# Alisah-Ozcan/HEonGPU

Measured on AMD Instinct MI355X. Metric: homomorphic mults/sec (CKKS N=2^16, L=16) + NTT GB/s vs HBM roofline, higher is better.
Workload: dtype u64

## Files before the change

heongpu_amd/csrc/ntt.hip:

```cpp
#include "ntt.hpp"
#define HEGPU_FP_TU ntt
#include "fpmod.cuh"

namespace hegpu {

#define NTT_THREADS 256

#ifdef NTT_ABLATION_HEADER
#include NTT_ABLATION_HEADER
#else
__device__ __forceinline__ u64 gld(const u64* p) { return *p; }
__device__ __forceinline__ void gst(u64* p, u64 v) { *p = v; }
#define NTT_ABLATE_BFLY(x, y, w)
#define NTT_ABLATE_FPBFLY(x, y, w)
#define NTT_ABLATE_TW(load, root0, s) (load)
#define NTT_FP_TW(t, i, c) ((t)[i])
#endif

__device__ __forceinline__ u64 csub(u64 x, u64 m) { return (x >= m) ? x - m : x; }

typedef unsigned long long u64x2_t __attribute__((ext_vector_type(2)));
struct ConstTw {
    const u64x2_t __attribute__((address_space(4)))* p;
    __device__ __forceinline__ ulonglong2 operator[](u32 i) const
// ... 883 lines not shown
            x[2 * k + 1] = v.y;
        }
        ct_radix16_tb<LAZY>(x, tb, qc);
        if (LAZY) {
#pragma unroll
            for (int k = 0; k < 16; k++) r[k] = reduce64(x[k], md);
        } else {
#pragma unroll
            for (int k = 0; k < 16; k++) r[k] = csub(csub(csub(x[k], qc.q4), 2 * qc.q), qc.q);
        }
    }
    wave_lds_fence();
#pragma unroll
    for (int k = 0; k < 8; k++)
        *reinterpret_cast<ulonglong2*>(&lds[row_phys(row * 256 + 16 * i0 + 2 * k)]) = make_ulonglong2(r[2 * k], r[2 * k + 1]);
    wave_lds_fence();
    row_store_all(a, ps, md, a.out + ps.out_off, (u64) g * 4096 + row * 256 + i0, lds, row, i0);
}

template <int S1, bool DECOMP = false>
__global__ __launch_bounds__(16 << S1, 4) void ntt_fwd_single(NttArgs a)
{
    extern __shared__ __attribute__((aligned(16))) u64 limb[];
    const PolySel ps = select_poly(a, blockIdx.x);
    if (DECOMP && a.skip_identity && ps.mod == ps.digit) return;
    const Mod md = a.mods[ps.mod];
    if (md.fp) fwd_single_body<S1, true, false, DECOMP>(a, ps, md, limb);
    else if (fwd_stages_lazy(md, a.lazy_q_max)) fwd_single_body<S1, false, true, DECOMP>(a, ps, md, limb);
    else fwd_single_body<S1, false, false, DECOMP>(a, ps, md, limb);
}

static_assert(ks_unreduced_exit(16, 60) == 16 && ks_unreduced_exit(17, 60) == 12 && ks_unreduced_exit(21, 60) == 12, "");
static_assert(ks_unreduced_exit(22, 60) == 8 && ks_unreduced_exit(32, 60) == 8 && ks_unreduced_exit(33, 60) == 0, "");
static_assert(ks_unreduced_exit(4, 61) == 16 && ks_unreduced_exit(8, 61) == 8 && ks_unreduced_exit(9, 61) == 0, "");

template <bool LAZY, int ROOM = 8, int EXIT = 0>
__device__ __forceinline__ void ks_row_digit(u64 (&x)[16], const u64* __restrict__ p, u64* lds,
                                             const ulonglong2* twa, const ulonglong2* __restrict__ tb,
                                             const QC& qc, const Mod& md, int row, int i0)
{
    static_assert(EXIT == 0 || (!LAZY && (EXIT == 8 || ((EXIT == 12 || EXIT == 16) && ROOM == 16))), "exit bound");
    constexpr CsSched CS = cs_sched(8, ROOM, EXIT ? EXIT : 8);
#pragma unroll
    for (int k = 0; k < 16; k++) x[k] = gld(&p[row * 256 + i0 + 16 * k]);
#pragma unroll
    for (int s = 0; s < 4; s++) {
        const int half = 8 >> s;
        const int cs = LAZY ? 0 : (int) (((CS.c8 >> s) & 1u) * 2u + ((CS.c4 >> s) & 1u));
#pragma unroll
        for (int b = 0; b < (1 << s); b++) {
            const ulonglong2 w = twa[((1 << s) - 1 + b) * 16 + row];
#pragma unroll
            for (int j = 0; j < half; j++) ct_bfly_cs(x[b * 2 * half + j], x[b * 2 * half + j + half], w, qc, cs);
        }
    }
#pragma unroll
    for (int k = 0; k < 16; k++) lds[row_phys(row * 256 + i0 + 16 * k)] = x[k];
    wave_lds_fence();
#pragma unroll
    for (int k = 0; k < 8; k++) {
        ulonglong2 v = *reinterpret_cast<const ulonglong2*>(&lds[row_phys(row * 256 + 16 * i0 + 2 * k)]);
        x[2 * k] = v.x;
        x[2 * k + 1] = v.y;
    }
    ct_radix16_tb<LAZY, (CS.c8 >> 4), (CS.c4 >> 4)>(x, tb, qc);
    if (!LAZY && EXIT == 0) {
#pragma unroll
        for (int k = 0; k < 16; k++) x[k] = csub(csub(csub(x[k], qc.q4), 2 * qc.q), qc.q);
    }
    wave_lds_fence();
#pragma unroll
    for (int k = 0; k < 8; k++)
        *reinterpret_cast<ulonglong2*>(&lds[row_phys(row * 256 + 16 * i0 + 2 * k)]) =
            make_ulonglong2(x[2 * k], x[2 * k + 1]);
    wave_lds_fence();
#pragma unroll
    for (int k = 0; k < 16; k++) x[k] = lds[row_phys(row * 256 + i0 + 16 * k)];
    wave_lds_fence();
}

struct KsIdx { int item, tile, slot; bool valid; int d0, d1; };
__host__ __device__ __forceinline__ unsigned ks_slots(const KsMacArgs& a, int kind)
{
    const int all = a.slot_count ? a.slot_count : a.rc;
    if (a.int_slot_count <= 0 || kind == 0) return (unsigned) all;
    return kind == 1 ? (unsigned) a.int_slot_count : (unsigned) (all - a.int_slot_count);
}
template <bool SPLIT, int KIND = 0>
__device__ __forceinline__ KsIdx ks_index(const KsMacArgs& a)
{
    const unsigned b = blockIdx.x, xcd = b & 7u, j = b >> 3;
    const unsigned splits = SPLIT ? (unsigned) a.splits : 1u;
    const unsigned units = (unsigned) a.items * splits;
    const unsigned tiles = 1u << (a.n_power - 12);
    const unsigned total = ks_slots(a, KIND) * tiles * units, chunk = (total + 7u) >> 3;
    const unsigned lin = xcd * chunk + j;
    const unsigned g = lin / units, unit = lin - g * units;
    const unsigned item = SPLIT ? unit / splits : unit, sp = SPLIT ? unit - item * splits : 0u;
    const unsigned nslots = ks_slots(a, KIND), gt = g / nslots;
    KsIdx r;
    r.valid = lin < total;
    r.item = (int) item;
    r.tile = (int) gt;
    int si = (int) (g - gt * nslots);
    if (KIND == 1 && a.int_slot_count > 0) {
        si = a.int_slots[r.valid ? si : 0];
    } else {
        si += a.slot_first;
        if (KIND == 2 && a.int_slot_count > 0) {
#pragma unroll
            for (int q = 0; q < 8; q++)
                if (q < a.int_slot_count && a.int_slots[q] <= si) si++;
        }
    }
    r.slot = si;
    r.d0 = SPLIT ? (int) (sp * (unsigned) a.digits / splits) : 0;
    r.d1 = SPLIT ? (int) ((sp + 1) * (unsigned) a.digits / splits) : a.digits;
    return r;
}

__device__ __forceinline__ void ks_tail_scatter(const KsMacArgs& a, int item, int slot, int p, u64 e0, const u64 (&r)[16])
{
    const KsMacArgs::Tail& e = a.tail;
    u64* out = e.out + e.out_item_stride * item + ((u64) (p * e.limbs + slot) << a.n_power);
    if (e.galois_inv) {
#pragma unroll
        for (int k = 0; k < 16; k++) {
            const u32 el = (u32) e0 + 16 * k;
            const u32 ex = ((2u * (__brev(el) >> (32 - a.n_power)) + 1u) * e.galois_inv) & ((2u << a.n_power) - 1u);
            out[__brev((ex - 1u) >> 1) >> (32 - a.n_power)] = r[k];
        }
    } else {
#pragma unroll
        for (int k = 0; k < 16; k++) out[e0 + 16 * k] = r[k];
    }
}
__device__ __forceinline__ void ks_tail_store(const KsMacArgs& a, int item, int slot, int p, u64 e0, const Mod& md, u64 inv,
                                              const u64 (&acc)[16], const u64 (&tv)[16], bool with_ct, const u64 (&cv)[16])
{
    u64 r[16];
#pragma unroll
    for (int k = 0; k < 16; k++) r[k] = mul_barrett(sub_mod(acc[k], tv[k], md.q), inv, md);
    if (with_ct) {
#pragma unroll
        for (int k = 0; k < 16; k++) r[k] = add_mod(cv[k], r[k], md.q);
    }
    ks_tail_scatter(a, item, slot, p, e0, r);
}
__device__ __forceinline__ void ks_tail_store_fp(const KsMacArgs& a, int item, int slot, int p, u64 e0, const FC& fc, double inv,
                                                 const double (&acc)[16], const double (&tv)[16], bool with_ct,
                                                 const u64 (&cv)[16])
{
    double m[16];
#pragma unroll
    for (int k = 0; k < 16; k++) {
        FP_STAGE(fc, FP_STAGE_OUT);
        const double d = fp_reduce(acc[k], fc) - tv[k];
        FP_STAGE(fc, FP_STAGE_TAIL);
        FP_AUDIT_VAL(fc, FPM_SUM, d);
        m[k] = fp_mul_nc(d, inv, fc);
    }
    FP_STAGE(fc, FP_STAGE_OUT);
    if (with_ct) {
#pragma unroll
        for (int k = 0; k < 16; k++) m[k] += fp_from_u64(cv[k]);
    }
    u64 r[16];
#pragma unroll
    for (int k = 0; k < 16; k++) r[k] = fp_to_u64(fp_canon(m[k], fc));
    ks_tail_scatter(a, item, slot, p, e0, r);
}
__device__ __forceinline__ const u64* ks_tail_T(const KsMacArgs& a, int item, int slot, int tile, int p)
{
    return a.tail.T + a.tail.T_item_stride * item + ((u64) (p * a.rc + slot) << a.n_power) + (u64) tile * 4096;
}
__device__ __forceinline__ bool ks_tail_ct(const KsMacArgs& a, int item, int slot, int p, u64 e0, u64 (&cv)[16])
{
    const KsMacArgs::Tail& e = a.tail;
    if (!e.ct || (e.ct_parts && p >= e.ct_parts)) return false;
    const u64* c = e.ct + e.ct_item_stride * item + ((u64) (p * e.limbs + slot) << a.n_power) + e0;
#pragma unroll
    for (int k = 0; k < 16; k++) cv[k] = c[16 * k];
    return true;
}

#define KS_TW_LDS_BYTES ((15 * 256 + 15 * 16) * 8)
template <bool SPLIT, bool MD = false>
__device__ __forceinline__ void ks_row_mac_int_body(const KsMacArgs& a, const KsIdx& ki, const Mod& md, int midx,
                                                    u64* lds, void* twbuf)
{
    const int t = threadIdx.x;
    const int item = ki.item, tile = ki.tile, slot = ki.slot;
    const QC qc = make_qc(md.q);
    const int s1 = a.n_power - 8;
    const ulonglong2* __restrict__ tw = a.tw + ((u64) midx << a.n_power);
    const int row = t >> 4, i0 = t & 15;
    const u32 crow = tile * 16 + row;
    const ulonglong2* __restrict__ tb = a.twB + ((u64) midx * (15u << (a.n_power - 4))) + ((u64) crow * 15 * 16 + i0);
    const u64 n = (u64) 1 << a.n_power;
    const u64* __restrict__ pin = a.in + a.in_item_stride * item + ((u64) slot << a.n_power) + (u64) tile * 4096;
    const u64* __restrict__ pk = a.key + ((u64) midx << a.n_power) + (u64) tile * 4096 + row * 256 + i0;
    const u64 dig_off = (u64) a.rc << a.n_power;
    const u64 key_off1 = (u64) a.key_limbs << a.n_power, key_off2 = (u64) a.key_limbs << (a.n_power + 1);
    const bool lazy = row_stages_lazy(md, a.lazy_q_max) && md.q <= ~0ull / (u64) a.digits;
    const bool room16 = stages_room16(md);
    const int ex = a.unreduced_exit;
    ulonglong2* twa = reinterpret_cast<ulonglong2*>(twbuf);
    if (i0 < 15) {
        const int s = (i0 >= 7) ? 3 : (i0 >= 3) ? 2 : (i0 >= 1) ? 1 : 0;
        twa[i0 * 16 + row] = tw[((((u32) 1 << s1) + crow) << s) + (i0 - ((1 << s) - 1))];
    }
    wave_lds_fence();

    const int item_s = MD ? __builtin_amdgcn_readfirstlane(item) : 0, slot_s = MD ? __builtin_amdgcn_readfirstlane(slot) : 0;
    const int tile_s = MD ? __builtin_amdgcn_readfirstlane(tile) : 0, midx_s = MD ? __builtin_amdgcn_readfirstlane(midx) : 0;
    u64 h0[16], l0[16], h1[16], l1[16];
#pragma unroll
    for (int k = 0; k < 16; k++) h0[k] = l0[k] = h1[k] = l1[k] = 0;
    for (int i = ki.d0; i < ki.d1; i++) {
        u64 x[16];
        const u64* p = pin + dig_off * i;
        if (a.skip_identity && i == midx) {
            const u64* pi = a.ident + a.ident_item_stride * item + ((u64) i << a.n_power) + (u64) tile * 4096;
#pragma unroll
            for (int k = 0; k < 16; k++) x[k] = gld(&pi[row * 256 + i0 + 16 * k]);
        } else if (lazy) {
            ks_row_digit<true>(x, p, lds, twa, tb, qc, md, row, i0);
        } else if (room16) {
            if (ex == 16) ks_row_digit<false, 16, 16>(x, p, lds, twa, tb, qc, md, row, i0);
            else if (ex == 12) ks_row_digit<false, 16, 12>(x, p, lds, twa, tb, qc, md, row, i0);
            else if (ex == 8) ks_row_digit<false, 16, 8>(x, p, lds, twa, tb, qc, md, row, i0);
            else ks_row_digit<false, 16>(x, p, lds, twa, tb, qc, md, row, i0);
        } else {
            if (ex) ks_row_digit<false, 8, 8>(x, p, lds, twa, tb, qc, md, row, i0);
            else ks_row_digit<false>(x, p, lds, twa, tb, qc, md, row, i0);
        }
        const u64* k0 = pk + key_off2 * i;
        const u64* k1 = k0 + key_off1;
#pragma unroll
        for (int k = 0; k < 16; k++) {
            acc128(h0[k], l0[k], x[k], k0[16 * k]);
            acc128(h1[k], l1[k], x[k], k1[16 * k]);
        }
    }
    if constexpr (MD) {
        u64 acc0[16], acc1[16];
#pragma unroll
        for (int k = 0; k < 16; k++) {
            acc0[k] = reduce128(h0[k], l0[k], md);
            acc1[k] = reduce128(h1[k], l1[k], md);
        }
        int tt = threadIdx.x;
        asm volatile("" : "+v"(tt));
        const int trow = tt >> 4, ti0 = tt & 15;
        const u64 e0 = (u64) tile_s * 4096 + trow * 256 + ti0;
        const u64 inv = a.tail.inv[midx_s];
        const bool lazy_t = row_stages_lazy(md, a.lazy_q_max);
        const ulonglong2* __restrict__ ttb = a.twB + ((u64) midx_s * (15u << (a.n_power - 4))) + ((u64) (tile_s * 16 + trow) * 15 * 16 + ti0);
        auto part = [&](int p, const u64 (&acc)[16]) {
            u64 cv[16], x[16];
            const bool with_ct = ks_tail_ct(a, item_s, slot_s, p, e0, cv);
            const u64* pT = ks_tail_T(a, item_s, slot_s, tile_s, p);
            if (lazy_t) {
                ks_row_digit<true>(x, pT, lds, twa, ttb, qc, md, trow, ti0);
#pragma unroll
                for (int k = 0; k < 16; k++) x[k] = reduce64(x[k], md);
            } else if (room16) {
                ks_row_digit<false, 16>(x, pT, lds, twa, ttb, qc, md, trow, ti0);
            } else {
                ks_row_digit<false>(x, pT, lds, twa, ttb, qc, md, trow, ti0);
            }
            ks_tail_store(a, item_s, slot_s, p, e0, md, inv, acc, x, with_ct, cv);
        };
        __builtin_amdgcn_sched_barrier(0);
        part(0, acc0);
        __builtin_amdgcn_sched_barrier(0);
        part(1, acc1);
        return;
    }
    u64* po = (SPLIT ? const_cast<u64*>(pin) + dig_off * ki.d0 - (u64) tile * 4096
                     : a.out + a.out_item_stride * item + ((u64) slot << a.n_power)) +
              (u64) tile * 4096 + row * 256 + i0;
#pragma unroll
    for (int k = 0; k < 16; k++) {
        po[16 * k] = reduce128(h0[k], l0[k], md);
        po[dig_off + 16 * k] = reduce128(h1[k], l1[k], md);
    }
    (void) n;
}

template <bool SPLIT>
__global__ __launch_bounds__(NTT_THREADS, SPLIT ? 2 : 1) void ks_row_mac(KsMacArgs a)
{
    __shared__ __attribute__((aligned(16))) u64 lds[ROW_LDS_ELEMS];
    __shared__ ulonglong2 twa[15 * 16];
    const KsIdx ki = ks_index<SPLIT, SPLIT ? 0 : 1>(a);
    if (!ki.valid) return;
    const int midx = a.mod_order ? a.mod_order[ki.slot] : ki.slot;
    const Mod md = a.mods[midx];
    if (md.fp) return;
    ks_row_mac_int_body<SPLIT>(a, ki, md, midx, lds, twa);
}

template <bool SPLIT>
__device__ __forceinline__ void ks_fp_row(double (&x)[16], const u64 (&xr)[16], const double* twl, u64* lds, const FC& fc,
                                          int s1, int row, int i0, int t)
{
    if constexpr (SPLIT) {
#pragma unroll
        for (int k = 0; k < 16; k++) x[k] = as_f64(xr[k]);
#pragma unroll
        for (int s = 0; s < 4; s++) {
            const int half = 8 >> s;
            FP_STAGE(fc, s1 + s);
#pragma unroll
            for (int b = 0; b < (1 << s); b++) {
                const double w = twl[15 * 256 + ((1 << s) - 1 + b) * 16 + row];
#pragma unroll
                for (int j = 0; j < half; j++) fp_ct_bfly(x[b * 2 * half + j], x[b * 2 * half + j + half], w, fc);
            }
        }
        FP_STAGE(fc, s1 + 4);
#pragma unroll
        for (int k = 0; k < 16; k++) x[k] = fp_reduce(x[k], fc);
#pragma unroll
        for (int k = 0; k < 16; k++) lds[row_phys(row * 256 + i0 + 16 * k)] = as_bits(x[k]);
        wave_lds_fence();
#pragma unroll
        for (int k = 0; k < 8; k++) {
            ulonglong2 v = *reinterpret_cast<const ulonglong2*>(&lds[row_phys(row * 256 + 16 * i0 + 2 * k)]);
            x[2 * k] = as_f64(v.x);
            x[2 * k + 1] = as_f64(v.y);
        }
#pragma unroll
        for (int s = 0; s < 4; s++) {
            const int half = 8 >> s;
            FP_STAGE(fc, s1 + 4 + s);
#pragma unroll
            for (int b = 0; b < (1 << s); b++) {
                const double w = twl[((1 << s) - 1 + b) * 256 + t];
#pragma unroll
                for (int j = 0; j < half; j++) fp_ct_bfly(x[b * 2 * half + j], x[b * 2 * half + j + half], w, fc);
            }
        }
    } else {
        int row_o = row, t_o = t;
        asm volatile("" : "+v"(row_o), "+v"(t_o));
        const double* twa = twl + 15 * 256 + row_o;
        const double* twb = twl + t_o;
        double wn[8], wc[8];
        wc[0] = twa[0];
        wn[0] = twa[16];
        wn[1] = twa[32];
        __builtin_amdgcn_sched_barrier(0);
#pragma unroll
        for (int k = 0; k < 16; k++) x[k] = as_f64(xr[k]);
#pragma unroll
        for (int s = 0; s < 4; s++) {
            const int half = 8 >> s;
            FP_STAGE(fc, s1 + s);
            if (s > 0) {
#pragma unroll
                for (int b = 0; b < (1 << s); b++) wc[b] = wn[b];
            }
            if (s < 3) {
                if (s > 0) {
#pragma unroll
                    for (int b = 0; b < (2 << s); b++) wn[b] = twa[((2 << s) - 1 + b) * 16];
                }
            } else {
                wn[0] = twb[0];
            }
            __builtin_amdgcn_sched_barrier(0);
#pragma unroll
            for (int b = 0; b < (1 << s); b++) {
                const double w = wc[b];
#pragma unroll
                for (int j = 0; j < half; j++) fp_ct_bfly(x[b * 2 * half + j], x[b * 2 * half + j + half], w, fc);
            }
        }
        FP_STAGE(fc, s1 + 4);
#pragma unroll
        for (int k = 0; k < 16; k++) x[k] = fp_reduce(x[k], fc);
#pragma unroll
        for (int k = 0; k < 16; k++) lds[row_phys(row * 256 + i0 + 16 * k)] = as_bits(x[k]);
        wave_lds_fence();
#pragma unroll
        for (int k = 0; k < 8; k++) {
            ulonglong2 v = *reinterpret_cast<const ulonglong2*>(&lds[row_phys(row * 256 + 16 * i0 + 2 * k)]);
            x[2 * k] = as_f64(v.x);
            x[2 * k + 1] = as_f64(v.y);
        }
#pragma unroll
        for (int s = 0; s < 4; s++) {
            const int half = 8 >> s;
            FP_STAGE(fc, s1 + 4 + s);
#pragma unroll
            for (int b = 0; b < (1 << s); b++) wc[b] = wn[b];
            if (s < 3) {
#pragma unroll
                for (int b = 0; b < (2 << s); b++) wn[b] = twb[((2 << s) - 1 + b) * 256];
            }
            __builtin_amdgcn_sched_barrier(0);
#pragma unroll
            for (int b = 0; b < (1 << s); b++) {
                const double w = wc[b];
#pragma unroll
                for (int j = 0; j < half; j++) fp_ct_bfly(x[b * 2 * half + j], x[b * 2 * half + j + half], w, fc);
            }
        }
    }
    wave_lds_fence();
#pragma unroll
    for (int k = 0; k < 8; k++)
        *reinterpret_cast<ulonglong2*>(&lds[row_phys(row * 256 + 16 * i0 + 2 * k)]) =
            make_ulonglong2(as_bits(x[2 * k]), as_bits(x[2 * k + 1]));
    wave_lds_fence();
#pragma unroll
    for (int k = 0; k < 16; k++) x[k] = as_f64(lds[row_phys(row * 256 + i0 + 16 * k)]);
    wave_lds_fence();
}

template <bool SPLIT, bool MD = false>
__device__ __forceinline__ void ks_row_mac_fp_body(const KsMacArgs& a, const KsIdx& ki, const Mod& md, int midx,
                                                   u64* lds, void* twbuf)
{
    const int t = threadIdx.x;
    const int item = ki.item, tile = ki.tile, slot = ki.slot;
    const FC fc = make_fc(md.q, FP_SITE(SPLIT ? FPS_KS_ROW_SPLIT : FPS_KS_ROW, a.n_power - 12));
    const int s1 = a.n_power - 8;
    const ulonglong2* __restrict__ tw = a.tw + ((u64) midx << a.n_power);
    const int row = t >> 4, i0 = t & 15;
    const u32 crow = tile * 16 + row;
    const double* __restrict__ tb8 = a.twB8 + ((u64) midx * (15u << (a.n_power - 4))) + ((u64) crow * 15 * 16 + i0);
    const u64* __restrict__ pin = a.in + a.in_item_stride * item + ((u64) slot << a.n_power) + (u64) tile * 4096;
    const u64* __restrict__ pk = a.key + ((u64) midx << a.n_power) + (u64) tile * 4096 + row * 256 + i0;
    const u64 dig_off = (u64) a.rc << a.n_power;
    const u64 key_off1 = (u64) a.key_limbs << a.n_power, key_off2 = (u64) a.key_limbs << (a.n_power + 1);

    double* twl = reinterpret_cast<double*>(twbuf);
#pragma unroll
    for (int k = 0; k < 15; k++) twl[k * 256 + t] = tb8[k * 16];
    if (i0 < 15) {
        const int s = (i0 >= 7) ? 3 : (i0 >= 3) ? 2 : (i0 >= 1) ? 1 : 0;
        const int b = i0 - ((1 << s) - 1);
        twl[15 * 256 + i0 * 16 + row] = as_f64(tw[((((u32) 1 << s1) + crow) << s) + b].x);
    }
    wave_lds_fence();

    const int item_s = MD ? __builtin_amdgcn_readfirstlane(item) : 0, slot_s = MD ? __builtin_amdgcn_readfirstlane(slot) : 0;
    const int tile_s = MD ? __builtin_amdgcn_readfirstlane(tile) : 0, midx_s = MD ? __builtin_amdgcn_readfirstlane(midx) : 0;
    double a0[16], a1[16];
#pragma unroll
    for (int k = 0; k < 16; k++) a0[k] = a1[k] = 0.0;
    int since = 0;
    for (int i = ki.d0; i < ki.d1; i++) {
        double x[16];
        const u64* p = pin + dig_off * i;
        const bool ident = a.skip_identity && i == midx;
        const u64* px = ident ? a.ident + a.ident_item_stride * item + ((u64) i << a.n_power) + (u64) tile * 4096 : p;
        u64 xr[16];
#pragma unroll
        for (int k = 0; k < 16; k++) {
            if constexpr (!SPLIT) xr[k] = __builtin_nontemporal_load(&px[row * 256 + i0 + 16 * k]);
            else xr[k] = px[row * 256 + i0 + 16 * k];
        }
        const u64* k0 = pk + key_off2 * i;
        const u64* k1 = k0 + key_off1;
        u64 kv0[16], kv1[16];
#pragma unroll
        for (int k = 0; k < 16; k++) {
            kv0[k] = k0[16 * k];
            kv1[k] = k1[16 * k];
        }
        if (ident) {
            FP_STAGE(fc, FP_STAGE_INPUT);
#pragma unroll
            for (int k = 0; k < 16; k++) x[k] = fp_reduce(fp_from_u64_ldexp(xr[k]), fc);
        } else {
            ks_fp_row<SPLIT>(x, xr, twl, lds, fc, s1, row, i0, t);
        }
#pragma unroll
        for (int k = 0; k < 16; k++) {
            FP_STAGE(fc, FP_STAGE_PRODUCT);
            a0[k] += fp_mul_nc(fp_from_u64_ldexp(kv0[k]), x[k], fc);
            a1[k] += fp_mul_nc(fp_from_u64_ldexp(kv1[k]), x[k], fc);
            FP_STAGE(fc, FP_STAGE_SUMS + since);
            FP_AUDIT_VAL(fc, FPM_SUM, a0[k]);
            FP_AUDIT_VAL(fc, FPM_SUM, a1[k]);
        }
        if (++since == 3) {
            since = 0;
            FP_STAGE(fc, FP_STAGE_SUMS + 3);
#pragma unroll
            for (int k = 0; k < 16; k++) {
                a0[k] = fp_reduce(a0[k], fc);
                a1[k] = fp_reduce(a1[k], fc);
            }
        }
    }
    if constexpr (MD) {
        int tt = threadIdx.x;
        asm volatile("" : "+v"(tt));
        const int trow = tt >> 4, ti0 = tt & 15;
        const u64 e0 = (u64) tile_s * 4096 + trow * 256 + ti0;
        const double inv = fp_from_u64(a.tail.inv[midx_s]);
        auto part = [&](int p, const double (&acc)[16]) {
            const u64* pT = ks_tail_T(a, item_s, slot_s, tile_s, p);
            u64 tr[16], cv[16];
#pragma unroll
            for (int k = 0; k < 16; k++) tr[k] = __builtin_nontemporal_load(&pT[trow * 256 + ti0 + 16 * k]);
            const bool with_ct = ks_tail_ct(a, item_s, slot_s, p, e0, cv);
            double x[16];
            ks_fp_row<false>(x, tr, twl, lds, fc, s1, trow, ti0, tt);
            ks_tail_store_fp(a, item_s, slot_s, p, e0, fc, inv, acc, x, with_ct, cv);
        };
        __builtin_amdgcn_sched_barrier(0);
        part(0, a0);
        __builtin_amdgcn_sched_barrier(0);
        part(1, a1);
        return;
    }
    u64* po = (SPLIT ? const_cast<u64*>(pin) + dig_off * ki.d0 - (u64) tile * 4096
                     : a.out + a.out_item_stride * item + ((u64) slot << a.n_power)) +
              (u64) tile * 4096 + row * 256 + i0;
    FP_STAGE(fc, FP_STAGE_OUT);
#pragma unroll
    for (int k = 0; k < 16; k++) {
        if constexpr (!SPLIT) {
            __builtin_nontemporal_store(fp_to_u64(fp_canon(a0[k], fc)), &po[16 * k]);
            __builtin_nontemporal_store(fp_to_u64(fp_canon(a1[k], fc)), &po[dig_off + 16 * k]);
        } else {
            po[16 * k] = fp_to_u64(fp_canon(a0[k], fc));
            po[dig_off + 16 * k] = fp_to_u64(fp_canon(a1[k], fc));
        }
    }
}

template <bool SPLIT>
__global__ __launch_bounds__(NTT_THREADS) void ks_row_mac_fp(KsMacArgs a)
{
    __shared__ __attribute__((aligned(16))) u64 lds[ROW_LDS_ELEMS];
    __shared__ double twl[15 * 256 + 15 * 16];
    const KsIdx ki = ks_index<SPLIT, SPLIT ? 0 : 2>(a);
    if (!ki.valid) return;
    const int midx = a.mod_order ? a.mod_order[ki.slot] : ki.slot;
    const Mod md = a.mods[midx];
    if (!md.fp) return;
    ks_row_mac_fp_body<SPLIT>(a, ki, md, midx, lds, twl);
}

__global__ __launch_bounds__(NTT_THREADS) void ks_row_mac_fp_moddown(KsMacArgs a)
{
    __shared__ __attribute__((aligned(16))) u64 lds[ROW_LDS_ELEMS];
    __shared__ double twl[15 * 256 + 15 * 16];
    const KsIdx ki = ks_index<false, 2>(a);
    if (!ki.valid) return;
    const int midx = a.mod_order ? a.mod_order[ki.slot] : ki.slot;
    const Mod md = a.mods[midx];
    if (!md.fp) return;
    ks_row_mac_fp_body<false, true>(a, ki, md, midx, lds, twl);
}
__global__ __launch_bounds__(NTT_THREADS, 1) void ks_row_mac_moddown(KsMacArgs a)
{
    __shared__ __attribute__((aligned(16))) u64 lds[ROW_LDS_ELEMS];
    __shared__ ulonglong2 twa[15 * 16];
    const KsIdx ki = ks_index<false, 1>(a);
    if (!ki.valid) return;
    const int midx = a.mod_order ? a.mod_order[ki.slot] : ki.slot;
    const Mod md = a.mods[midx];
    if (md.fp) return;
    ks_row_mac_int_body<false, true>(a, ki, md, midx, lds, twa);
}

__global__ __launch_bounds__(NTT_THREADS, 2) void ks_row_mac_split(KsMacArgs a)
{
    __shared__ __attribute__((aligned(16))) u64 lds[ROW_LDS_ELEMS];
    __shared__ double twl[15 * 256 + 15 * 16];
    const KsIdx ki = ks_index<true>(a);
    if (!ki.valid) return;
    const int midx = a.mod_order ? a.mod_order[ki.slot] : ki.slot;
    const Mod md = a.mods[midx];
    if (md.fp) ks_row_mac_fp_body<true>(a, ki, md, midx, lds, twl);
    else ks_row_mac_int_body<true>(a, ki, md, midx, lds, twl);
}

hipError_t ks_row_mac_launch(const KsMacArgs& a, int items, hipStream_t st)
{
    if (a.digits > 64 || items <= 0) return hipErrorInvalidValue;
    if (a.splits > 1 && a.digits < 2 * a.splits) return hipErrorInvalidValue;
    if (a.tail.on && (a.splits > 1 || !a.tail.out || !a.tail.T || !a.tail.inv)) return hipErrorInvalidValue;
    if (a.slot_first < 0 || a.slot_count < 0 || a.slot_first + (a.slot_count ? a.slot_count : a.rc) > a.rc)
        return hipErrorInvalidValue;
    KsMacArgs k = a;
    k.items = items;
    if (k.int_slot_count < 0 || k.int_slot_count > 8) k.int_slot_count = 0;
    const unsigned tiles = (1u << a.n_power) / 4096, units = (unsigned) items * (a.splits > 1 ? (unsigned) a.splits : 1u);
    auto grid_of = [&](int kind) { return dim3(8u * ((ks_slots(k, kind) * tiles * units + 7u) / 8u)); };
    if (a.splits > 1) {
        hipLaunchKernelGGL(ks_row_mac_split, grid_of(0), dim3(NTT_THREADS), 0, st, k);
    } else {
        if (!a.no_fp && ks_slots(k, 2) > 0) {
            if (a.tail.on) hipLaunchKernelGGL(ks_row_mac_fp_moddown, grid_of(2), dim3(NTT_THREADS), 0, st, k);
            else hipLaunchKernelGGL(ks_row_mac_fp<false>, grid_of(2), dim3(NTT_THREADS), 0, st, k);
        }
        if (!a.no_int && ks_slots(k, 1) > 0) {
            if (a.tail.on) hipLaunchKernelGGL(ks_row_mac_moddown, grid_of(1), dim3(NTT_THREADS), 0, st, k);
            else hipLaunchKernelGGL(ks_row_mac<false>, grid_of(1), dim3(NTT_THREADS), 0, st, k);
        }
    }
    return hipGetLastError();
}

__device__ __forceinline__ void fp_gs_bfly(double& x, double& y, ulonglong2 w, const FC& c)
{
    const double s = x + y, d = x - y;
    x = s;
    y = fp_mul(d, as_f64(w.x), as_f64(w.y), c);
    FP_AUDIT_VAL(c, FPM_SUM, s);
}

struct ArInt {
    typedef u64 T;
    QC qc;
    __device__ __forceinline__ explicit ArInt(const Mod& md) : qc(make_qc(md.q)) {}
    __device__ __forceinline__ T from_canon(u64 v) const { return v; }
    __device__ __forceinline__ T from_bits(u64 v) const { return v; }
    __device__ __forceinline__ u64 to_bits(T v) const { return v; }
    template <int LOGR>
    __device__ __forceinline__ void radix(T (&x)[1 << LOGR], const ulonglong2* __restrict__ tw, u32 root0) const
    {
        gs_radix<LOGR>(x, tw, root0, qc);
    }
    __device__ __forceinline__ void radix16_tb(T (&x)[16], const ulonglong2* __restrict__ tb) const { gs_radix16_tb(x, tb, qc); }
    template <int LOGR>
    __device__ __forceinline__ void radix_last(T (&x)[1 << LOGR], const ulonglong2* __restrict__ tw, ulonglong2 ninv,
                                               ulonglong2 w1ninv, u64 (&out)[1 << LOGR]) const
    {
        gs_radix_last<LOGR>(x, tw, 1u, ninv, w1ninv, qc);
#pragma unroll
        for (int k = 0; k < (1 << LOGR); k++) out[k] = x[k];
    }
};

struct ArFp {
    typedef double T;
    FC fc;
    int s1;
    __device__ __forceinline__ explicit ArFp(const Mod& md, int n_power) : fc(make_fc(md.q, FP_SITE(FPS_INV, n_power - 12))), s1(n_power - 8) {}
    __device__ __forceinline__ T from_canon(u64 v) const { return fp_from_u64(v); }
    __device__ __forceinline__ T from_bits(u64 v) const { return as_f64(v); }
    __device__ __forceinline__ u64 to_bits(T v) const { return as_bits(v); }
    template <int N>
    __device__ __forceinline__ void reduce_all(T (&x)[N]) const
    {
#pragma unroll
        for (int k = 0; k < N; k++) x[k] = fp_reduce(x[k], fc);
    }
    template <int LOGR>
    __device__ __forceinline__ void radix(T (&x)[1 << LOGR], const ulonglong2* __restrict__ tw, u32 root0) const
    {
        int done = 0;
#pragma unroll
        for (int s = LOGR - 1; s >= 0; s--) {
            const int half = (1 << LOGR) >> (s + 1);
            FP_STAGE(fc, 31 - __builtin_clz(root0) + s);
#pragma unroll
            for (int b = 0; b < (1 << s); b++) {
                const ulonglong2 w = tw[(root0 << s) + b];
#pragma unroll
                for (int j = 0; j < half; j++) fp_gs_bfly(x[b * 2 * half + j], x[b * 2 * half + j + half], w, fc);
            }
            if ((++done & 1) == 0 || s == 0) reduce_all(x);
        }
    }
    __device__ __forceinline__ void radix16_tb(T (&x)[16], const ulonglong2* __restrict__ tb) const
    {
#pragma unroll
        for (int s = 3; s >= 0; s--) {
            const int half = 8 >> s;
            FP_STAGE(fc, s1 + 4 + s);
#pragma unroll
            for (int b = 0; b < (1 << s); b++) {
                const ulonglong2 w = tb[((1 << s) - 1 + b) * 16];
#pragma unroll
                for (int j = 0; j < half; j++) fp_gs_bfly(x[b * 2 * half + j], x[b * 2 * half + j + half], w, fc);
            }
            if (s == 2 || s == 0) reduce_all(x);
        }
    }
    template <int LOGR>
    __device__ __forceinline__ void radix_last(T (&x)[1 << LOGR], const ulonglong2* __restrict__ tw, ulonglong2 ninv,
                                               ulonglong2 w1ninv, u64 (&out)[1 << LOGR]) const
    {
        int done = 0;
#pragma unroll
        for (int s = LOGR - 1; s >= 1; s--) {
            const int half = (1 << LOGR) >> (s + 1);
            FP_STAGE(fc, s);
#pragma unroll
            for (int b = 0; b < (1 << s); b++) {
                const ulonglong2 w = tw[(1u << s) + b];
#pragma unroll
                for (int j = 0; j < half; j++) fp_gs_bfly(x[b * 2 * half + j], x[b * 2 * half + j + half], w, fc);
            }
            if ((++done & 1) == 0) reduce_all(x);
        }
        constexpr int half = (1 << LOGR) >> 1;
        FP_STAGE(fc, 0);
#pragma unroll
        for (int j = 0; j < half; j++) {
            const double sum = x[j] + x[j + half], d = x[j] - x[j + half];
            out[j] = fp_to_u64(fp_canon(fp_mul(sum, as_f64(ninv.x), as_f64(ninv.y), fc), fc));
            out[j + half] = fp_to_u64(fp_canon(fp_mul(d, as_f64(w1ninv.x), as_f64(w1ninv.y), fc), fc));
        }
    }
};

template <typename AR, bool TO_LDS, bool TENSOR = false>
__device__ __forceinline__ void inv_row_part(const AR& ar, const NttArgs& a, int mod, int tt, u32 crow0,
                                             const u64* __restrict__ src, u64* __restrict__ dst, u64* lds,
                                             int tensor_part = 0)
{
    typedef typename AR::T T;
    const int s1 = a.n_power - 8;
    const ulonglong2* __restrict__ tw = a.itw + ((u64) mod << a.n_power);
    const int row = tt >> 4, i0 = tt & 15;
    const u32 crow = crow0 + row;
    if (TENSOR) {
        const Mod md = a.mods[mod];
        const u64 part_off = (u64) a.tensor_limbs << a.n_power;
        const u64* __restrict__ a0 = src, * __restrict__ a1 = src + part_off, * __restrict__ b0 = src + 2 * part_off,
                 * __restrict__ b1 = src + 3 * part_off;
#pragma unroll
        for (int k0 = 0; k0 < 16; k0 += 4) {
            u64 r[4];
            if (tensor_part == 1) {
                u64 va0[4], va1[4], vb0[4], vb1[4];
#pragma unroll
                for (int k = 0; k < 4; k++) {
                    const int e = row * 256 + i0 + 16 * (k0 + k);
                    va0[k] = a0[e]; va1[k] = a1[e]; vb0[k] = b0[e]; vb1[k] = b1[e];
                }
#pragma unroll
                for (int k = 0; k < 4; k++) {
                    u64 h1, l1, h2, l2;
                    mul64wide(va0[k], vb1[k], h1, l1);
                    mul64wide(va1[k], vb0[k], h2, l2);
                    const u64 lo = l1 + l2;
                    r[k] = reduce128(h1 + h2 + (lo < l1), lo, md);
                }
            } else {
                const u64* __restrict__ pa = tensor_part == 0 ? a0 : a1;
                const u64* __restrict__ pb = tensor_part == 0 ? b0 : b1;
                u64 va[4], vb[4];
#pragma unroll
                for (int k = 0; k < 4; k++) {
                    const int e = row * 256 + i0 + 16 * (k0 + k);
                    va[k] = pa[e]; vb[k] = pb[e];
                }
#pragma unroll
                for (int k = 0; k < 4; k++) r[k] = mul_barrett(va[k], vb[k], md);
            }
#pragma unroll
            for (int k = 0; k < 4; k++) lds[row_phys(row * 256 + i0 + 16 * (k0 + k))] = r[k];
        }
    } else {
#pragma unroll
        for (int k = 0; k < 16; k++) lds[row_phys(row * 256 + i0 + 16 * k)] = gld(&src[row * 256 + i0 + 16 * k]);
    }
    wave_lds_fence();
    T x[16];
#pragma unroll
    for (int k = 0; k < 8; k++) {
        ulonglong2 v = *reinterpret_cast<const ulonglong2*>(&lds[row_phys(row * 256 + 16 * i0 + 2 * k)]);
        x[2 * k] = ar.from_canon(v.x);
        x[2 * k + 1] = ar.from_canon(v.y);
    }
    ar.radix16_tb(x, a.itwB + ((u64) mod * (15u << (a.n_power - 4))) + ((u64) crow * 15 * 16 + i0));
    wave_lds_fence();
#pragma unroll
    for (int k = 0; k < 8; k++)
        *reinterpret_cast<ulonglong2*>(&lds[row_phys(row * 256 + 16 * i0 + 2 * k)]) =
            make_ulonglong2(ar.to_bits(x[2 * k]), ar.to_bits(x[2 * k + 1]));
    wave_lds_fence();
#pragma unroll
    for (int k = 0; k < 16; k++) x[k] = ar.from_bits(lds[row_phys(row * 256 + i0 + 16 * k)]);
    ar.template radix<4>(x, tw, (1u << s1) + crow);
    if constexpr (TO_LDS) {
#pragma unroll
        for (int k = 0; k < 16; k++) lds[row_phys(row * 256 + i0 + 16 * k)] = ar.to_bits(x[k]);
    } else {
#pragma unroll
        for (int k = 0; k < 16; k++) gst(&dst[row * 256 + i0 + 16 * k], ar.to_bits(x[k]));
    }
}

struct InvEpi {
    const u64* last;
    const u64* ct;
    u64* out;
    Mod md;
    u64 half, qP, hm, inv;
    int galois, n_power;
    bool pre;
};
__device__ __forceinline__ bool inv_epi_setup(const NttArgs& a, const PolySel& ps, InvEpi& e, bool& skip)
{
    skip = false;
    if (!a.iepi.on) return false;
    const NttInvEpilogue& ep = a.iepi;
    const int pc = ep.p_count ? ep.p_count : 1;
    const int part = udiv16(ps.j, ep.mg_slots), limb = ps.j - part * (ep.limbs + pc);
    if (limb >= ep.limbs) { skip = true; return true; }
    const u64 item_in = a.out_item_stride * ps.item;
    const u64 off = (u64) (part * ep.limbs + limb) << a.n_power;
    e.pre = ep.u != nullptr;
// ... 580 lines not shown
```

Baseline: 8960.

## Prefetch next digit tile into LDS via async global_load_lds in key-switch MAC

In the non-split FP key-switch row MAC, the input digit tile is now fetched with asynchronous global-to-LDS DMA loads, with a swizzled layout. The next digit's tile (or the tail T tile) is issued while the current digit's products are computed. Each thread then reads its row from LDS after waiting on vmcnt. The aim is to hide global load latency behind the FP MAC work, at the cost of LDS traffic, explicit waitcnt fences and reuse of the LDS buffer shared with the row NTT.

```diff
diff --git a/heongpu_amd/csrc/ntt.hip b/heongpu_amd/csrc/ntt.hip
--- a/heongpu_amd/csrc/ntt.hip
+++ b/heongpu_amd/csrc/ntt.hip
@@ -1209,6 +1209,42 @@
     ks_row_mac_int_body<SPLIT>(a, ki, md, midx, lds, twa);
 }
 
+__device__ __forceinline__ void ks_tile_dma(const u64* src, u64* lds, int t)
+{
+    const u32 w = __builtin_amdgcn_readfirstlane(t >> 6), l = t & 63;
+    const u32 voff = (w * 1024 + 2 * (l ^ ((l >> 4) & 3))) * 8;
+    const u64 sb = (u64) src;
+    const u32 sb_lo = (u32) __builtin_amdgcn_readfirstlane((u32) sb), sb_hi = (u32) __builtin_amdgcn_readfirstlane((u32) (sb >> 32));
+    const char* base = reinterpret_cast<const char*>(((u64) sb_hi << 32) | (u64) sb_lo);
+    typedef __attribute__((address_space(1))) const void* gptr_t;
+    typedef __attribute__((address_space(3))) void* lptr_t;
+#pragma unroll
+    for (int h = 0; h < 2; h++) {
+        const char* bh = base + h * 4096;
+        asm volatile("" : "+s"(bh));
+        const gptr_t ge = (gptr_t) (bh + voff), go = (gptr_t) (bh + (voff ^ 64u));
+        const lptr_t ld = (lptr_t) (lds + w * 1024 + h * 512);
+        __builtin_amdgcn_global_load_lds(ge, ld, 16, 0, 2);
+        __builtin_amdgcn_global_load_lds(go, ld, 16, 1024, 2);
+        __builtin_amdgcn_global_load_lds(ge, ld, 16, 2048, 2);
+        __builtin_amdgcn_global_load_lds(go, ld, 16, 3072, 2);
+    }
+}
+__device__ __forceinline__ void ks_dma_issue_fence()
+{
+    __builtin_amdgcn_sched_barrier(0);
+    asm volatile("s_waitcnt lgkmcnt(0)" ::: "memory");
+}
+__device__ __forceinline__ void ks_tile_take(u64 (&xr)[16], const u64* lds, int row, int i0)
+{
+    __builtin_amdgcn_sched_barrier(0);
+    asm volatile("s_waitcnt vmcnt(0)" ::: "memory");
+#pragma unroll
+    for (int k = 0; k < 16; k++) xr[k] = lds[row_phys(row * 256 + i0 + 16 * k)];
+    wave_lds_fence();
+    __builtin_amdgcn_sched_barrier(0);
+}
+
 template <bool SPLIT>
 __device__ __forceinline__ void ks_fp_row(double (&x)[16], const u64 (&xr)[16], const double* twl, u64* lds, const FC& fc,
                                           int s1, int row, int i0, int t)
@@ -1346,6 +1382,14 @@
     const u64 key_off1 = (u64) a.key_limbs << a.n_power, key_off2 = (u64) a.key_limbs << (a.n_power + 1);
 
     double* twl = reinterpret_cast<double*>(twbuf);
+    auto digit_src = [&](int i) -> const u64* {
+        return (a.skip_identity && i == midx) ? a.ident + a.ident_item_stride * item + ((u64) i << a.n_power) + (u64) tile * 4096
+                                              : pin + dig_off * i;
+    };
+    if constexpr (!SPLIT) {
+        if (ki.d0 < ki.d1) ks_tile_dma(digit_src(ki.d0), lds, t);
+        else if constexpr (MD) ks_tile_dma(ks_tail_T(a, item, slot, tile, 0), lds, t);
+    }
 #pragma unroll
     for (int k = 0; k < 15; k++) twl[k * 256 + t] = tb8[k * 16];
     if (i0 < 15) {
@@ -1363,14 +1407,14 @@
     int since = 0;
     for (int i = ki.d0; i < ki.d1; i++) {
         double x[16];
-        const u64* p = pin + dig_off * i;
         const bool ident = a.skip_identity && i == midx;
-        const u64* px = ident ? a.ident + a.ident_item_stride * item + ((u64) i << a.n_power) + (u64) tile * 4096 : p;
         u64 xr[16];
-#pragma unroll
-        for (int k = 0; k < 16; k++) {
-            if constexpr (!SPLIT) xr[k] = __builtin_nontemporal_load(&px[row * 256 + i0 + 16 * k]);
-            else xr[k] = px[row * 256 + i0 + 16 * k];
+        if constexpr (SPLIT) {
+            const u64* px = digit_src(i);
+#pragma unroll
+            for (int k = 0; k < 16; k++) xr[k] = px[row * 256 + i0 + 16 * k];
+        } else {
+            ks_tile_take(xr, lds, row, i0);
         }
         const u64* k0 = pk + key_off2 * i;
         const u64* k1 = k0 + key_off1;
@@ -1387,11 +1431,24 @@
         } else {
             ks_fp_row<SPLIT>(x, xr, twl, lds, fc, s1, row, i0, t);
         }
+        double kd0[16], kd1[16];
+        if constexpr (!SPLIT) {
+#pragma unroll
+            for (int k = 0; k < 16; k++) {
+                kd0[k] = fp_from_u64_ldexp(kv0[k]);
+                kd1[k] = fp_from_u64_ldexp(kv1[k]);
+                asm volatile("" : "+v"(kd0[k]), "+v"(kd1[k]));
+            }
+            ks_dma_issue_fence();
+            const u64* nxt = (i + 1 < ki.d1) ? digit_src(i + 1) : MD ? ks_tail_T(a, item_s, slot_s, tile_s, 0) : nullptr;
+            if (MD || i + 1 < ki.d1) ks_tile_dma(nxt, lds, t);
+            __builtin_amdgcn_sched_barrier(0);
+        }
 #pragma unroll
         for (int k = 0; k < 16; k++) {
             FP_STAGE(fc, FP_STAGE_PRODUCT);
-            a0[k] += fp_mul_nc(fp_from_u64_ldexp(kv0[k]), x[k], fc);
-            a1[k] += fp_mul_nc(fp_from_u64_ldexp(kv1[k]), x[k], fc);
+            a0[k] += fp_mul_nc(SPLIT ? fp_from_u64_ldexp(kv0[k]) : kd0[k], x[k], fc);
+            a1[k] += fp_mul_nc(SPLIT ? fp_from_u64_ldexp(kv1[k]) : kd1[k], x[k], fc);
             FP_STAGE(fc, FP_STAGE_SUMS + since);
             FP_AUDIT_VAL(fc, FPM_SUM, a0[k]);
             FP_AUDIT_VAL(fc, FPM_SUM, a1[k]);
@@ -1413,13 +1470,20 @@
         const u64 e0 = (u64) tile_s * 4096 + trow * 256 + ti0;
         const double inv = fp_from_u64(a.tail.inv[midx_s]);
         auto part = [&](int p, const double (&acc)[16]) {
-            const u64* pT = ks_tail_T(a, item_s, slot_s, tile_s, p);
             u64 tr[16], cv[16];
-#pragma unroll
-            for (int k = 0; k < 16; k++) tr[k] = __builtin_nontemporal_load(&pT[trow * 256 + ti0 + 16 * k]);
+            ks_tile_take(tr, lds, trow, ti0);
             const bool with_ct = ks_tail_ct(a, item_s, slot_s, p, e0, cv);
             double x[16];
             ks_fp_row<false>(x, tr, twl, lds, fc, s1, trow, ti0, tt);
+            if (p == 0) {
+                if (with_ct) {
+#pragma unroll
+                    for (int k = 0; k < 16; k++) asm volatile("" : "+v"(cv[k]));
+                }
+                ks_dma_issue_fence();
+                ks_tile_dma(ks_tail_T(a, item_s, slot_s, tile_s, 1), lds, tt);
+                __builtin_amdgcn_sched_barrier(0);
+            }
             ks_tail_store_fp(a, item_s, slot_s, p, e0, fc, inv, acc, x, with_ct, cv);
         };
         __builtin_amdgcn_sched_barrier(0);
```

Measured after the change: 8999, median of 6. No clear change (+0.4%).
